# NVIDIA-Genomics-Research/GenomeWorks

Measured on AMD Instinct MI355X. Metric: cudapoa consensus GCUPS, 1024-window short-read batch (static band 256, 32 reads <= 1024 bp), higher is better.
Workload: dtype int16; 1 GPU; BASELINE configs[2]: cudapoa single-batch consensus, 1024 windows x 32 reads, backbone 960 bp, <=48 sub/24 ins/24 del, BatchConfig(1024,32,256,static_band), scores 8/-6/-8; windows_per_gpu=1024, cells_per_gpu=10990578176, parallelism=index-split x1

## Files before the change

genomeworks_amd/csrc/gwhip_poa.hip:

```cpp
#include <hip/hip_runtime.h>

#include <cstdio>
#include <cstdlib>
#include <cstring>
#include <string>

#include "poa_device.h"
#include "poa_full_device.h"
#include "poa_graph_device.h"
#include "poa_tb_device.h"

namespace gwhip
{

#ifndef GWHIP_POA_PART
thread_local std::string g_last_error;

static int fail(hipError_t e, const char* what)
{
    g_last_error = std::string(what) + ": " + hipGetErrorString(e);
    return (int)e;
}
static int fail_msg(int code, const std::string& msg)
{
// ... 177 lines not shown
        }
    }
    if (lane == 0) consensus[0] = 0;
    uint64_t cells = 0;
    int32_t node_count = len0;
    uint64_t phase_acc[kPhCount] = {0, 0, 0, 0, 0, 0};
    PhaseClock pc{(DBG && a.phase_cycles) ? phase_acc : nullptr, 0};
    wave_sync();
    pc.start();

    for (int32_t s = 1; s < (int32_t)wd.num_seqs; s++)
    {
        const int32_t seq_len = seq_lens[s];
        const int32_t adv     = ((s == 1 ? len0 : seq_lens[s - 1]) + 3) & ~3;
        sequence += adv;
        base_weights += adv;

        if (node_count >= c.max_nodes_per_graph)
        {
            if (lane == 0) { consensus[0] = kKernelError; consensus[1] = kNodeCountExceeded; }
            break;
        }
        pc.tick(kPhOther);
        build_rowinfo<IdT, RowT>(g, node_count, rowinfo, lane, LDS_TABLES ? reinterpret_cast<uint64_t*>(lds_code_tile) : nullptr);
        constexpr bool LDS_READ = LDS_TABLES && BM != GWHIP_FULL_BAND;
        const uint8_t* lds_read = lds_read_buf;
        if constexpr (LDS_READ)
        {
            typedef uint32_t StageVec __attribute__((ext_vector_type(4)));
            typedef StageVec StageVecA4 __attribute__((aligned(4)));
            static_assert(kReadLds % 16 == 0 && (kRingBytes + kRowInfoBytes) % 16 == 0, "16-byte fetches fill the LDS copy of the read");
            const int32_t stage_bytes = min(kReadLds, ((max(seq_len, kMaxAdaptiveBand) + 8) + 3) & ~3);
            for (int32_t i = lane * 16; i < stage_bytes; i += kWave * 16)
                *reinterpret_cast<StageVec*>(lds_read_buf + i) = *reinterpret_cast<const StageVecA4*>(sequence + i);
        }
        wave_sync();
        pc.tick(kPhRowInfo);
        const uint8_t* banded_read = LDS_READ ? lds_read : sequence;

        int32_t alen = 0;
        constexpr bool kTbPacked = TB && LDS_TABLES && std::is_same<ScoreT, int16_t>::value && std::is_same<TraceT, int16_t>::value;
        bool tb_handled = false;
        if constexpr (kTbPacked)
        {
            constexpr bool kAd = BM == GWHIP_ADAPTIVE_BAND_TRACEBACK;
            const bool adaptive_now = kAd && c.alignment_band_width < kMaxAdaptiveBand;
            auto packed = [&](auto ad_tag, int32_t rerun) -> int32_t {
// ... 20 lines not shown
            else
            alen = nw_banded_tb<ScoreT, IdT, RowT, TraceT, true>(g, rowinfo, node_count, sequence, seq_len, scores, a.L.scores_elems,
                                                           traceback, a.L.trace_elems, banded_buffer_size, alignment_graph,
                                                           alignment_read, c.alignment_band_width, c.max_banded_pred_distance,
                                                           c.gap_score, c.mismatch_score, c.match_score, 0, cells);
            if (alen == kShiftLeft || alen == kShiftRight)
                alen = nw_banded_tb<ScoreT, IdT, RowT, TraceT, true>(g, rowinfo, node_count, sequence, seq_len, scores, a.L.scores_elems,
                                                               traceback, a.L.trace_elems, banded_buffer_size, alignment_graph,
                                                               alignment_read, c.alignment_band_width, c.max_banded_pred_distance,
                                                               c.gap_score, c.mismatch_score, c.match_score, alen, cells);
        }
        else if (TB)
        {
            alen = nw_banded_tb<ScoreT, IdT, RowT, TraceT, false>(g, rowinfo, node_count, sequence, seq_len, scores, a.L.scores_elems,
                                                            traceback, a.L.trace_elems, banded_buffer_size, alignment_graph,
                                                            alignment_read, c.alignment_band_width, c.max_banded_pred_distance,
                                                            c.gap_score, c.mismatch_score, c.match_score, 0, cells);
        }
        else if (BM == GWHIP_ADAPTIVE_BAND && c.alignment_band_width < kMaxAdaptiveBand)
        {
            alen = nw_banded<ScoreT, IdT, RowT, true, LDS_READ, PV>(g, rowinfo, node_count, banded_read, lds_read, seq_len, scores, ring, ring_bytes,
                                                banded_buffer_size, alignment_graph, alignment_read, c.alignment_band_width,
                                                c.gap_score, c.mismatch_score, c.match_score, 0, cells, pc, debug_flags, codes, lds_code_tile, lds_read_window, lds_bs_ring,
                                                mw_args, mw_shared);
            if (alen == kShiftLeft || alen == kShiftRight)
                alen = nw_banded<ScoreT, IdT, RowT, true, LDS_READ, PV>(g, rowinfo, node_count, banded_read, lds_read, seq_len, scores, ring, ring_bytes,
                                                    banded_buffer_size, alignment_graph, alignment_read,
                                                    c.alignment_band_width, c.gap_score, c.mismatch_score, c.match_score,
                                                    alen, cells, pc, debug_flags, codes, lds_code_tile, lds_read_window, lds_bs_ring,
                                                    mw_args, mw_shared);
        }
        else if (BM == GWHIP_STATIC_BAND || BM == GWHIP_ADAPTIVE_BAND)
        {
            alen = nw_banded<ScoreT, IdT, RowT, false, LDS_READ, PV>(g, rowinfo, node_count, banded_read, lds_read, seq_len, scores, ring, ring_bytes,
                                                 banded_buffer_size, alignment_graph, alignment_read, c.alignment_band_width,
                                                 c.gap_score, c.mismatch_score, c.match_score, 0, cells, pc, debug_flags, codes, lds_code_tile, lds_read_window, lds_bs_ring);
        }
        else
        {
            bool full_handled = false;
            if constexpr (kFullPacked)
                alen = nw_full_packed<IdT>(g, rowinfo, node_count, sequence, seq_len, reinterpret_cast<int16_t*>(scores), wd.scores_width, full_moves,
                                           smem, kRingBytes, reinterpret_cast<const uint64_t*>(lds_code_tile), alignment_graph, alignment_read,
                                           c.gap_score, c.mismatch_score, c.match_score, cells, debug_flags, full_handled, pc);
            if (!full_handled)
                alen = nw_full<ScoreT, IdT, RowT>(g, rowinfo, node_count, sequence, seq_len, scores, wd.scores_width, ring, kRingBytes,
                                            alignment_graph, alignment_read, c.gap_score, c.mismatch_score, c.match_score, cells);
        }
        alen = (int32_t)(IdT)alen;

        uint8_t err = 0;
        if (alen == kNwLoopFailed) err = kLoopCountExceeded;
        else if (alen == kNwAdaptiveStorageFailed) err = kExceededAdaptiveBandedMatrixSize;
        else if (TB && alen == kNwTracebackBufferFailed) err = kExceededMaximumPredecessorDistance;
        else if (alen == kNwPipelineFailed || alen == kNwScoreWrapped) err = kGenericError;
        if (err)
        {
            if (lane == 0) { consensus[0] = kKernelError; consensus[1] = err; }
            break;
// ... 640 lines not shown
```

genomeworks_amd/csrc/poa_device.h:

```cpp
#pragma once
#include <hip/hip_runtime.h>
#include <stdint.h>

#include <type_traits>

#include "poa_layout.h"
#include "poa_pred_rows.h"

namespace gwhip
{

constexpr int kWave = 64;

template <typename T> struct Limits;
template <> struct Limits<int16_t> { static constexpr int32_t min = -32768; };
template <> struct Limits<int32_t> { static constexpr int32_t min = INT32_MIN; };

template <typename ScoreT> struct alignas(sizeof(ScoreT) * 4) Quad { ScoreT v[4]; };

template <typename ScoreT> __device__ __forceinline__ int32_t narrow_chk(int32_t v, bool& wrapped)
{
    const int32_t n = (int32_t)(ScoreT)v;
    if constexpr (sizeof(ScoreT) == 2) wrapped |= n != v;
    return n;
}

template <bool PACKED> struct RowInfo;
template <> struct alignas(8) RowInfo<true>
{
    uint64_t w;
// ... 689 lines not shown
    const uint64_t t_pp = psel == 6 ? clock64() : 0;
    if (aligned_nodes > 0 && (aligned_nodes & (kStage - 1)) != 0)
        flush_stage(aligned_nodes & ~(kStage - 1), aligned_nodes & (kStage - 1));
    if ((dbg & 2) && prof_acc && lane == 0) *prof_acc += (uint64_t)max(aligned_nodes, 0);
    if (aligned_nodes >= bound) aligned_nodes = kNwLoopFailed;
    wave_sync();
    for (int32_t k0 = lane; k0 < aligned_nodes; k0 += 4 * kWave)
    {
        int32_t pos[4], node[4];
#pragma unroll
        for (int u = 0; u < 4; u++) pos[u] = (k0 + u * kWave < aligned_nodes) ? alignment_graph[k0 + u * kWave] : -1;
#pragma unroll
        for (int u = 0; u < 4; u++) node[u] = (int32_t)g.sorted_poa[max(pos[u], 0)];
#pragma unroll
        for (int u = 0; u < 4; u++)
            if (pos[u] >= 0) alignment_graph[k0 + u * kWave] = node[u];
    }
    wave_sync();
    if (psel == 6) pacc += clock64() - t_pp;
    if (psel && lane == 0) *prof_acc += pacc;
    return aligned_nodes;
}

template <typename IdT, typename RowT>
__device__ __forceinline__ void build_rowinfo(const GraphView<IdT>& g, int32_t graph_count, RowT* rowinfo, int lane,
                                              uint64_t* xpred = nullptr)
{
    if (xpred != nullptr)
    {
#pragma unroll
        for (int q = 0; q < 4; q++) xpred[q * kWave + lane] = 0;
        wave_sync();
    }
    if (lane == 0) rowinfo[0].set(0, 0, false, 0, 0, 0);
    constexpr int kU = 4;
    for (int32_t r0 = 1 + lane; r0 <= graph_count; r0 += kU * kWave)
    {
        int32_t node[kU], cnt[kU], oc[kU], bas[kU], e0[kU], e1[kU], e2[kU], q0[kU], q1[kU], q2[kU];
        int32_t e3[kU], e4[kU], e5[kU], q3[kU] = {}, q4[kU] = {}, q5[kU] = {};
#pragma unroll
        for (int u = 0; u < kU; u++) node[u] = g.sorted_poa[min(r0 + u * kWave, graph_count) - 1];
#pragma unroll
        for (int u = 0; u < kU; u++)
        {
            cnt[u] = g.incoming_edge_count[node[u]];
            oc[u]  = g.outgoing_edge_count[node[u]];
            bas[u] = g.nodes[node[u]];
            e0[u]  = g.incoming_edges[(int64_t)node[u] * kEdges + 0];
            e1[u]  = g.incoming_edges[(int64_t)node[u] * kEdges + 1];
            e2[u]  = g.incoming_edges[(int64_t)node[u] * kEdges + 2];
        }
#pragma unroll
        for (int u = 0; u < kU; u++)
        {
            q0[u] = g.node_id_to_pos[(uint32_t)e0[u] < (uint32_t)graph_count ? e0[u] : 0];
            q1[u] = g.node_id_to_pos[(uint32_t)e1[u] < (uint32_t)graph_count ? e1[u] : 0];
            q2[u] = g.node_id_to_pos[(uint32_t)e2[u] < (uint32_t)graph_count ? e2[u] : 0];
            e3[u] = e4[u] = e5[u] = 0;
            if (xpred != nullptr && cnt[u] > 3)
            {
                e3[u] = g.incoming_edges[(int64_t)node[u] * kEdges + 3];
                e4[u] = g.incoming_edges[(int64_t)node[u] * kEdges + 4];
                e5[u] = g.incoming_edges[(int64_t)node[u] * kEdges + 5];
            }
        }
        if (xpred != nullptr)
        {
            bool any = false;
#pragma unroll
            for (int u = 0; u < kU; u++) any |= cnt[u] > 3;
            if (__ballot(any) != 0)
            {
#pragma unroll
                for (int u = 0; u < kU; u++)
                {
                    q3[u] = q4[u] = q5[u] = 0;
                    if (cnt[u] > 3)
                    {
                        q3[u] = g.node_id_to_pos[(uint32_t)e3[u] < (uint32_t)graph_count ? e3[u] : 0];
                        q4[u] = g.node_id_to_pos[(uint32_t)e4[u] < (uint32_t)graph_count ? e4[u] : 0];
                        q5[u] = g.node_id_to_pos[(uint32_t)e5[u] < (uint32_t)graph_count ? e5[u] : 0];
                    }
                }
            }
        }
#pragma unroll
        for (int u = 0; u < kU; u++)
        {
            const int32_t r = r0 + u * kWave;
            if (r <= graph_count)
            {
                RowT ri{};
                ri.set(bas[u], cnt[u], oc[u] == 0, cnt[u] > 0 ? q0[u] + 1 : 0, cnt[u] > 1 ? q1[u] + 1 : 0, cnt[u] > 2 ? q2[u] + 1 : 0);
                rowinfo[r] = ri;
                if (xpred != nullptr && cnt[u] > 3)
                    xpred[r & (kSideTableSlots - 1)] = xpred_entry(r, cnt[u], q3[u] + 1, q4[u] + 1, q5[u] + 1);
            }
        }
    }
}

template <typename ScoreT, typename IdT>
__device__ __forceinline__ void banded_forward_1pass(const GraphView<IdT>& g, const RowInfo<true>* rowinfo,
                                                     int32_t graph_count, const uint8_t* lds_read, ScoreT* scores,
                                                     ScoreT* ring, int32_t ring_rows, int32_t band_width,
                                                     int32_t max_column, int32_t gap_score, int32_t mismatch_score,
                                                     int32_t match_score, int32_t dbg, uint64_t* general_row_acc, bool& wrapped)
{
    const int lane          = threadIdx.x & (kWave - 1);
    const int32_t min_score = Limits<ScoreT>::min / 2;
    const int32_t stride    = band_width + kRightPad;
    const int32_t lane4     = lane * 4;
    uint64_t general_acc    = 0;
    const bool full_wave    = band_width == 256;
    const bool active       = lane4 < band_width;
    const int32_t K0 = (lane4 + 0) * gap_score, K1 = (lane4 + 1) * gap_score, K2 = (lane4 + 2) * gap_score,
                  K3 = (lane4 + 3) * gap_score;
    int32_t P0 = K0 + gap_score, P1 = K1 + gap_score, P2 = K2 + gap_score, P3 = K3 + gap_score;
    int32_t prev_bs = 0, prev_rel0 = 0;
    int32_t ring_slot = 0;
    bool hbm_dirty    = false;
    ScoreT* row_out   = scores;
// ... 814 lines not shown
        if ((uint32_t)tg < (uint32_t)band_width)
        {
            const int32_t rel = tg + 1;
            const int32_t slot_r = slot_now();
            lds_st_quad<ScoreT>(ring + slot_r * stride + rel + kRelShift, (ScoreT)H0, (ScoreT)H1, (ScoreT)H2, (ScoreT)H3);
            global_st_quad<ScoreT>(scores + (int64_t)r * stride + rel + kRelShift, (ScoreT)H0, (ScoreT)H1, (ScoreT)H2, (ScoreT)H3);
            if (codes) *reinterpret_cast<__attribute__((address_space(1))) uint32_t*>(codes + (int64_t)r * stride + rel + kRelShift) = code4;
        }
        if (first_block && lane == 0)
        {
            *(__attribute__((address_space(3))) ScoreT*)(ring + slot_now() * stride + kRelShift) = (ScoreT)rel0_val;
            scores[(int64_t)r * stride + kRelShift]                                          = (ScoreT)rel0_val;
        }
        publish(r, __builtin_amdgcn_readlane(H3, kWave - 1));
        if (sksel == 8 || (sksel == 11 && first_block)) skacc += clock64() - t_rb;
    }
    }
    if (sksel == 4) skacc += clock64() - t_pass;
    if (sksel && lane == 0) __hip_atomic_fetch_add(&shared->prof, (unsigned long long)skacc, __ATOMIC_RELAXED, __HIP_MEMORY_SCOPE_WORKGROUP);
    block_barrier();
    if (sksel && prof_out && lane == 0) *prof_out += shared->prof;
}

template <typename ScoreT, typename IdT, typename RowT, bool ADAPTIVE, bool LDS_READ, int PV = 0>
__device__ __forceinline__ int32_t nw_banded(const GraphView<IdT>& g, RowT* rowinfo, int32_t graph_count, const uint8_t* read,
                             const uint8_t* lds_read, int32_t read_length, ScoreT* scores, ScoreT* ring_base, int32_t ring_bytes,
                             float max_buffer_size, int32_t* alignment_graph, int32_t* alignment_read,
                             int32_t band_width, int32_t gap_score, int32_t mismatch_score, int32_t match_score,
                             int32_t rerun, uint64_t& cells, PhaseClock& pc, int32_t dbg = 0, uint8_t* codes = nullptr,
                             uint8_t* code_tile = nullptr, uint8_t* read_window = nullptr, int32_t* bs_ring = nullptr,
                             MwArgs<ScoreT>* mw_args = nullptr, MwShared* mw_shared = nullptr)
{
    const int lane              = threadIdx.x & (kWave - 1);
    const int32_t min_score     = Limits<ScoreT>::min / 2;
    const float gradient        = __fdiv_rn((float)(read_length + 1), (float)(graph_count + 1));
    const int32_t max_column    = read_length + 1;

    if (ADAPTIVE)
    {
        if ((double)gradient > 1.1)
            band_width = max(band_width, ((int32_t)((double)max_column * 0.08 * (double)gradient) + 127) & ~127);
        if ((double)gradient < 0.8)
            band_width = max(band_width, ((int32_t)((double)max_column * 0.1 / (double)gradient) + 127) & ~127);
        band_width = min(band_width, kMaxAdaptiveBand);
        if (band_width == kMaxAdaptiveBand && rerun != 0) return rerun;
    }
    int32_t band_shift = band_width / 2;
    if (ADAPTIVE)
    {
        if (rerun == kShiftLeft && band_width <= kMaxAdaptiveBand / 2)
        {
            band_width *= 2;
            band_shift = (int32_t)((double)band_shift * 2.5);
        }
        if (rerun == kShiftRight && band_width <= kMaxAdaptiveBand / 2)
        {
            band_width *= 2;
            band_shift = (int32_t)((double)band_shift * 1.5);
        }
        float required = __fmul_rn((float)graph_count, (float)(band_width + kRightPad));
        if (required > max_buffer_size) return kNwAdaptiveStorageFailed;
    }
    cells += (uint64_t)graph_count * (uint64_t)band_width;

    BandedCtx<ScoreT> b;
    b.scores     = scores;
    b.stride     = band_width + kRightPad;
    b.band_width = band_width;
    b.band_shift = band_shift;
    b.max_column = max_column;
    b.gradient   = gradient;
    b.min_score  = min_score;
    b.ring       = ring_base;
    b.ring_rows  = ring_bytes / (int32_t)(b.stride * sizeof(ScoreT));
    if (b.ring_rows < 2) b.ring_rows = 0;
    if (bs_ring != nullptr) b.ring_rows = min(b.ring_rows, 64);
    const int32_t stride = b.stride;
    const int32_t npass  = (band_width + 255) / 256;
    const bool reg_path  = (npass == 1);

    for (int32_t rel = lane; rel <= band_width; rel += kWave)
    {
        ScoreT v = (ScoreT)(rel * gap_score);
        scores[rel + kRelShift] = v;
        if (b.ring_rows) b.ring[rel + kRelShift] = v;
    }
    int32_t P0 = 0, P1 = 0, P2 = 0, P3 = 0;
    int32_t prev_bs   = 0;
    int32_t prev_rel0 = 0;
    if (reg_path)
    {
        int32_t c = 4 * lane;
        P0 = (ScoreT)((c + 1) * gap_score);
        P1 = (ScoreT)((c + 2) * gap_score);
        P2 = (ScoreT)((c + 3) * gap_score);
        P3 = (ScoreT)((c + 4) * gap_score);
        prev_rel0 = 0;
    }
    for (int32_t r = 1 + lane; r <= graph_count; r += kWave)
        rowinfo[r].set_bs(band_start_for_row(r, gradient, band_width, band_shift, max_column));
    bool hbm_dirty = true;
    wave_sync();
    hbm_dirty = false;
    auto bs_of = [&](int32_t row, int32_t r) -> int32_t {
        if (row == 0) return 0;
        if (bs_ring && b.ring_rows && r - row < b.ring_rows) return bs_ring[row % b.ring_rows];
        return uniform_row(rowinfo[row]).bs();
    };
    constexpr int32_t kWin = 4096, kWinStep = 1024;
    int32_t staged_end = 0;
    auto stage_read = [&](int32_t need_end) {
        while (staged_end < need_end)
        {
            for (int32_t i = lane * 4; i < kWinStep; i += kWave * 4)
            {
                const int32_t col = staged_end + i;
                const uint32_t v = col < read_length + 8 ? *reinterpret_cast<const uint32_t*>(read + col) : 0u;
                *reinterpret_cast<uint32_t*>(read_window + (col & (kWin - 1))) = v;
            }
            staged_end += kWinStep;
        }
        wave_sync();
    };

    constexpr bool kFastOk = std::is_same<RowT, RowInfo<true>>::value && LDS_READ;
    bool fast_done = false, codes_valid = false, moves_valid = false;
    bool packed_selective = false;
    bool wrapped = false;
    if constexpr (kFastOk && std::is_same<ScoreT, int16_t>::value)
    {
        const bool width_ok  = PV == 2 ? (band_width == 384 || band_width == 512) : (band_width == 256 || (PV == 1 && band_width == 128));
        const int32_t u_span = max(band_width, 256) * abs(gap_score);
        const bool packed_ok = width_ok && max_column >= band_width && ring_bytes >= kPkSlots * kPkSlotBytes &&
                               abs(gap_score) <= 30 && abs(match_score) <= 100 && abs(mismatch_score) <= 100 &&
                               codes != nullptr && !(dbg & 256) && ring_bytes >= kMtBytes &&
                               max(match_score, 0) * min(read_length, graph_count) + u_span + abs(match_score) <= 32767 &&
                               (graph_count + read_length) * min(min(gap_score, mismatch_score), 0) >= -32768 + 256 &&
                               min_score + 4 * min(min(gap_score, mismatch_score), 0) - u_span >= -32768;
        static_assert(kWdSlots * kWdSlotBytes <= kPkSlots * kPkSlotBytes, "the two-pass ring lives in the 256-column pass's ring region");
        if (packed_ok)
        {
            if constexpr (PV == 2)
            {
                if (band_width == 384)
                    banded_forward_moves_wide<IdT, 384>(g, rowinfo, graph_count, lds_read, scores, codes, reinterpret_cast<uint8_t*>(ring_base),
                                                        reinterpret_cast<const uint64_t*>(code_tile), max_column, gap_score, mismatch_score, match_score, dbg);
                else
                    banded_forward_moves_wide<IdT, 512>(g, rowinfo, graph_count, lds_read, scores, codes, reinterpret_cast<uint8_t*>(ring_base),
                                                        reinterpret_cast<const uint64_t*>(code_tile), max_column, gap_score, mismatch_score, match_score, dbg);
            }
            else if (band_width == 256)
            {
                banded_forward_moves<IdT, 256>(g, rowinfo, graph_count, lds_read, scores, codes, reinterpret_cast<uint8_t*>(ring_base),
                                               reinterpret_cast<const uint64_t*>(code_tile), max_column, gap_score, mismatch_score, match_score,
                                               dbg, pc.acc ? &pc.acc[kPhOther] : nullptr, (dbg & (1 << 25)) != 0);
                packed_selective = !(dbg & (1 << 25));
            }
            else if constexpr (PV == 1)
            {
                banded_forward_moves<IdT, 128>(g, rowinfo, graph_count, lds_read, scores, codes, reinterpret_cast<uint8_t*>(ring_base),
                                               reinterpret_cast<const uint64_t*>(code_tile), max_column, gap_score, mismatch_score, match_score,
                                               dbg, pc.acc ? &pc.acc[kPhOther] : nullptr, (dbg & (1 << 25)) != 0);
                packed_selective = !(dbg & (1 << 25));
            }
            fast_done   = true;
            moves_valid = true;
        }
    }
    if constexpr (kFastOk)
    {
        if (!fast_done && npass == 1 && b.ring_rows >= 2)
        {
            banded_forward_1pass<ScoreT, IdT>(g, rowinfo, graph_count, lds_read, scores, b.ring, b.ring_rows, band_width,
                                              max_column, gap_score, mismatch_score, match_score, dbg,
                                              pc.acc ? &pc.acc[kPhOther] : nullptr, wrapped);
            fast_done = true;
        }
    }
    if constexpr (!std::is_same<RowT, RowInfo<true>>::value)
    {
        const int32_t sk_rows = min(b.ring_rows, (int32_t)(200.0f / (gradient + 1.0f)));
        if (!fast_done && mw_args != nullptr && npass >= 2 && sk_rows >= kSkLead + 3 && !(dbg & (1 << 18)))
        {
            MwArgs<ScoreT> A;
            A.op = 1;
// ... 331 lines not shown
```

genomeworks_amd/csrc/poa_forward_moves.h:

```cpp
#pragma once

#include "poa_forward_row_operands.h"

namespace gwhip
{

constexpr int kKindShift = 60;
constexpr uint32_t kMoveHoriz = 1;

__device__ __forceinline__ uint32_t pk_mad_u16_vsv(uint32_t a, uint32_t s, uint32_t c)
{
    uint32_t d;
    asm("v_pk_mad_u16 %0, %1, %2, %3" : "=v"(d) : "v"(a), "s"(s), "v"(c));
    return d;
}
__device__ __forceinline__ uint32_t pk_mad_u16_vvs(uint32_t a, uint32_t b, uint32_t s)
{
    uint32_t d;
    asm("v_pk_mad_u16 %0, %1, %2, %3" : "=v"(d) : "v"(a), "v"(b), "s"(s));
    return d;
}
__device__ __forceinline__ void gstore_nt_u64(void* p, uint32_t lo, uint32_t hi)
{
    u32x2 v;
// ... 93 lines not shown
            {
                int32_t e[kB], q[kB];
#pragma unroll
                for (int u = 0; u < kB; u++) e[u] = (int32_t)g.incoming_edges[edges + min(k0 + u, cnt - 1)];
#pragma unroll
                for (int u = 0; u < kB; u++) q[u] = (int32_t)g.node_id_to_pos[e[u]];
#pragma unroll
                for (int u = 0; u < kB; u++) mark(q[u] + 1);
            }
        }
    }
    wave_sync();
}
__device__ __forceinline__ bool row_recompute_safe(uint64_t w)
{
    return ((uint32_t)(w >> kKindShift) & 7u) >= 4u || ((w >> 8) & 0x3fu) > 3u || ((w >> 15) & 0x1ffu) == 0u;
}

template <typename IdT, int BW>
__device__ __forceinline__ void banded_forward_moves(const GraphView<IdT>& g, RowInfo<true>* rowinfo, int32_t graph_count,
                                                     const uint8_t* lds_read, int16_t* scores, uint8_t* moves, uint8_t* ring,
                                                     const uint64_t* xpred, int32_t max_column, int32_t gap_score,
                                                     int32_t mismatch_score, int32_t match_score, int32_t dbg,
                                                     uint64_t* prof_acc, bool store_all = true)
{
    const bool abl       = (dbg & (1 << 14)) != 0;
    const bool st_scores = !(abl && (dbg & (1 << 26))), st_moves = !(abl && (dbg & (1 << 27)));
    const bool ab_ring = !(abl && (dbg & (1 << 20))), ab_guard = !(abl && (dbg & (1 << 19))), ab_scan = !(abl && (dbg & (1 << 18))),
               ab_moves = !(abl && (dbg & (1 << 17))), ab_rows = !(abl && (dbg & (1 << 16)));
    const int32_t ksel = prof_acc ? ((dbg >> 28) & 7) - 1 : -1;
    const bool kfine   = (dbg & (1 << 13)) != 0;
    const bool kcount  = (dbg & (1 << 12)) != 0;
    uint64_t kacc      = 0;
    auto kselected = [&](uint32_t dk) -> bool { return ksel == (int32_t)((kfine || dk < kDkRingThree) ? dk : (uint32_t)kDkRingTwo); };
    const bool ksel_prev = kselected(kDkPrev), ksel_moved = kselected(kDkPrevMoved), ksel_one = kselected(kDkRingOne),
               ksel_two = kselected(kDkRingTwo), ksel_three = kselected(kDkRingThree), ksel_many = kselected(kDkRingMany),
               ksel_general = kselected(kDkGeneral);
    static_assert(kRowOpSlots == kPkSlots && kRowOpSlotBytes == kPkSlotBytes, "the row operands fold the ring's geometry in");
    static_assert(BW == 128 || BW == 256, "band widths of the packed pass");
    constexpr int32_t band_width = BW;
    constexpr int32_t stride     = band_width + kRightPad;
    constexpr int kBandLanes     = BW / kCellsPerLane;
    const int lane               = threadIdx.x & (kWave - 1);
    const bool band_lane         = lane < kBandLanes;
    const int32_t lane4 = lane * 4, lane8 = lane * 8;
    const int32_t min_score = Limits<int16_t>::min / 2;

    const bool time_prologue  = prof_acc != nullptr && ksel < 0 && kcount;
    const uint64_t t_prologue = time_prologue ? clock64() : 0;
    const int32_t first_moved = classify_kinds(rowinfo, graph_count, lane, xpred, dbg);
    wave_sync();
    static_assert(kPkSlots * kPkSlotBytes >= 4096 * (int)sizeof(uint16_t), "the ring region holds the list of left-over rows (rows <= 4095)");
    mark_score_rows<IdT>(g, rowinfo, graph_count, lane, store_all, reinterpret_cast<uint16_t*>(ring), xpred);
    if (time_prologue && lane == 0) *prof_acc += clock64() - t_prologue;

    const uint32_t MIN2   = pin_vgpr(pk_dup(min_score));
    const uint32_t SENT2  = pin_vgpr(pk_dup(kPkSentinel));
    const uint32_t GAP2   = pin_vgpr(pk_dup(gap_score));
    const uint32_t MAT2   = pin_vgpr(pk_dup(match_score));
    const uint32_t DIF2   = pin_vgpr(pk_dup(mismatch_score - match_score));
    const uint32_t ONE2   = pin_vgpr(0x00010001u);
    const uint32_t THREE2 = pin_vgpr(0x00030003u);
    const uint32_t NEG1   = pin_vgpr(0xffffffffu);
    const uint32_t K01 = pk_make((lane4 + 0) * gap_score, (lane4 + 1) * gap_score);
    const uint32_t K23 = pk_make((lane4 + 2) * gap_score, (lane4 + 3) * gap_score);
    const uint32_t ring_base = lds_addr(ring);
    const uint32_t read_base = lds_addr(lds_read);
    const uint32_t guard_off  = lane < 16 ? (uint32_t)(2 * BW) : (lane == 16 ? (uint32_t)-136 : (uint32_t)(120 - 16 * lane));
    const bool is_lane16      = lane == 16;
    const bool is_lane63      = lane == kBandLanes - 1;
    const uint32_t move_keep  = lane == 0 ? 0xffffff00u : 0xffffffffu;
    const uint32_t GUARD_HI_MIN = pin_vgpr(is_lane16 ? (((uint32_t)kPkSentinel & 0xffffu) | ((uint32_t)min_score << 16)) : pk_dup(kPkSentinel));
    const uint32_t S0X_MIN      = (uint32_t)min_score << 16;

    uint32_t P01 = pk_make((lane4 + 1) * gap_score, (lane4 + 2) * gap_score);
    uint32_t P23 = pk_make((lane4 + 3) * gap_score, (lane4 + 4) * gap_score);
// ... 434 lines not shown
```

Measured before the change: 451.1 GCUPS.

## Fold row classification and score-row marking into the row-table build

When the static or adaptive banded int16 packed pass will run, the row table is built in a new pass that also computes each row's band start, its kind and its mark bit, and collects a list of rows whose predecessors need marking. The forward-moves kernel then skips its separate classify_kinds and mark_score_rows prologue passes. This saves two extra sweeps over the row table plus their wave syncs for each read. In exchange it duplicates the classification rules in a new header, which must stay in step with the original, and it adds atomic ORs into the LDS row words.

```diff
diff --git a/genomeworks_amd/csrc/gwhip_poa.hip b/genomeworks_amd/csrc/gwhip_poa.hip
--- a/genomeworks_amd/csrc/gwhip_poa.hip
+++ b/genomeworks_amd/csrc/gwhip_poa.hip
@@ -223,7 +223,26 @@
             break;
         }
         pc.tick(kPhOther);
-        build_rowinfo<IdT, RowT>(g, node_count, rowinfo, lane, LDS_TABLES ? reinterpret_cast<uint64_t*>(lds_code_tile) : nullptr);
+        constexpr bool kFinishTable = LDS_TABLES && std::is_same<ScoreT, int16_t>::value && PV <= 1 &&
+                                      (BM == GWHIP_STATIC_BAND || BM == GWHIP_ADAPTIVE_BAND);
+        RowTableFinish fin{};
+        if constexpr (kFinishTable)
+        {
+            const bool adaptive_now = BM == GWHIP_ADAPTIVE_BAND && c.alignment_band_width < kMaxAdaptiveBand;
+            fin.plan = adaptive_now ? band_plan<true>(node_count, seq_len, c.alignment_band_width, 0, banded_buffer_size)
+                                    : band_plan<false>(node_count, seq_len, c.alignment_band_width, 0, banded_buffer_size);
+            const bool finish = fin.plan.early == 0 && !row_table_old_passes(debug_flags) && fin.plan.max_column <= kFinishMaxColumn &&
+                                packed_pass_ok<PV>(fin.plan.band_width, fin.plan.max_column, seq_len, node_count, ring_bytes, c.gap_score,
+                                                   c.mismatch_score, c.match_score, codes != nullptr, debug_flags);
+            const bool time_stores = pc.acc != nullptr && (debug_flags & (7 << 28)) == 0 && (debug_flags & (3 << 12)) == (3 << 12);
+            if (__builtin_amdgcn_readfirstlane((int32_t)finish) != 0)
+                build_rowinfo_finished<IdT>(g, node_count, rowinfo, lane, reinterpret_cast<uint64_t*>(lds_code_tile), reinterpret_cast<uint64_t*>(smem),
+                                            fin, time_stores ? &pc.acc[kPhOther] : nullptr);
+            else
+                build_rowinfo<IdT, RowT>(g, node_count, rowinfo, lane, reinterpret_cast<uint64_t*>(lds_code_tile));
+        }
+        else
+            build_rowinfo<IdT, RowT>(g, node_count, rowinfo, lane, LDS_TABLES ? reinterpret_cast<uint64_t*>(lds_code_tile) : nullptr);
         constexpr bool LDS_READ = LDS_TABLES && BM != GWHIP_FULL_BAND;
         const uint8_t* lds_read = lds_read_buf;
         if constexpr (LDS_READ)
@@ -290,7 +309,7 @@
             alen = nw_banded<ScoreT, IdT, RowT, true, LDS_READ, PV>(g, rowinfo, node_count, banded_read, lds_read, seq_len, scores, ring, ring_bytes,
                                                 banded_buffer_size, alignment_graph, alignment_read, c.alignment_band_width,
                                                 c.gap_score, c.mismatch_score, c.match_score, 0, cells, pc, debug_flags, codes, lds_code_tile, lds_read_window, lds_bs_ring,
-                                                mw_args, mw_shared);
+                                                mw_args, mw_shared, kFinishTable ? &fin : nullptr);
             if (alen == kShiftLeft || alen == kShiftRight)
                 alen = nw_banded<ScoreT, IdT, RowT, true, LDS_READ, PV>(g, rowinfo, node_count, banded_read, lds_read, seq_len, scores, ring, ring_bytes,
                                                     banded_buffer_size, alignment_graph, alignment_read,
@@ -302,7 +321,8 @@
         {
             alen = nw_banded<ScoreT, IdT, RowT, false, LDS_READ, PV>(g, rowinfo, node_count, banded_read, lds_read, seq_len, scores, ring, ring_bytes,
                                                  banded_buffer_size, alignment_graph, alignment_read, c.alignment_band_width,
-                                                 c.gap_score, c.mismatch_score, c.match_score, 0, cells, pc, debug_flags, codes, lds_code_tile, lds_read_window, lds_bs_ring);
+                                                 c.gap_score, c.mismatch_score, c.match_score, 0, cells, pc, debug_flags, codes, lds_code_tile, lds_read_window, lds_bs_ring,
+                                                 nullptr, nullptr, kFinishTable ? &fin : nullptr);
         }
         else
         {
diff --git a/genomeworks_amd/csrc/poa_device.h b/genomeworks_amd/csrc/poa_device.h
--- a/genomeworks_amd/csrc/poa_device.h
+++ b/genomeworks_amd/csrc/poa_device.h
@@ -6,6 +6,7 @@
 
 #include "poa_layout.h"
 #include "poa_pred_rows.h"
+#include "poa_row_finish.h"
 
 namespace gwhip
 {
@@ -741,6 +742,63 @@
     return aligned_nodes;
 }
 
+constexpr int kRowChunks = 4;
+struct RowChunkLoads
+{
+    int32_t cnt[kRowChunks], oc[kRowChunks], bas[kRowChunks];
+    int32_t q0[kRowChunks], q1[kRowChunks], q2[kRowChunks], q3[kRowChunks], q4[kRowChunks], q5[kRowChunks];
+};
+template <typename IdT>
+__device__ __forceinline__ void load_row_chunks(const GraphView<IdT>& g, int32_t graph_count, int32_t r0, bool side, RowChunkLoads& L)
+{
+    constexpr int kU = kRowChunks;
+    int32_t node[kU], e0[kU], e1[kU], e2[kU], e3[kU], e4[kU], e5[kU];
+#pragma unroll
+    for (int u = 0; u < kU; u++) node[u] = g.sorted_poa[min(r0 + u * kWave, graph_count) - 1];
+#pragma unroll
+    for (int u = 0; u < kU; u++)
+    {
+        L.cnt[u] = g.incoming_edge_count[node[u]];
+        L.oc[u]  = g.outgoing_edge_count[node[u]];
+        L.bas[u] = g.nodes[node[u]];
+        e0[u]    = g.incoming_edges[(int64_t)node[u] * kEdges + 0];
+        e1[u]    = g.incoming_edges[(int64_t)node[u] * kEdges + 1];
+        e2[u]    = g.incoming_edges[(int64_t)node[u] * kEdges + 2];
+    }
+#pragma unroll
+    for (int u = 0; u < kU; u++)
+    {
+        L.q0[u] = g.node_id_to_pos[(uint32_t)e0[u] < (uint32_t)graph_count ? e0[u] : 0];
+        L.q1[u] = g.node_id_to_pos[(uint32_t)e1[u] < (uint32_t)graph_count ? e1[u] : 0];
+        L.q2[u] = g.node_id_to_pos[(uint32_t)e2[u] < (uint32_t)graph_count ? e2[u] : 0];
+        e3[u] = e4[u] = e5[u] = 0;
+        L.q3[u] = L.q4[u] = L.q5[u] = 0;
+        if (side && L.cnt[u] > 3)
+        {
+            e3[u] = g.incoming_edges[(int64_t)node[u] * kEdges + 3];
+            e4[u] = g.incoming_edges[(int64_t)node[u] * kEdges + 4];
+            e5[u] = g.incoming_edges[(int64_t)node[u] * kEdges + 5];
+        }
+    }
+    if (side)
+    {
+        bool any = false;
+#pragma unroll
+        for (int u = 0; u < kU; u++) any |= L.cnt[u] > 3;
+        if (__ballot(any) != 0)
+        {
+#pragma unroll
+            for (int u = 0; u < kU; u++)
+                if (L.cnt[u] > 3)
+                {
+                    L.q3[u] = g.node_id_to_pos[(uint32_t)e3[u] < (uint32_t)graph_count ? e3[u] : 0];
+                    L.q4[u] = g.node_id_to_pos[(uint32_t)e4[u] < (uint32_t)graph_count ? e4[u] : 0];
+                    L.q5[u] = g.node_id_to_pos[(uint32_t)e5[u] < (uint32_t)graph_count ? e5[u] : 0];
+                }
+        }
+    }
+}
+
 template <typename IdT, typename RowT>
 __device__ __forceinline__ void build_rowinfo(const GraphView<IdT>& g, int32_t graph_count, RowT* rowinfo, int lane,
                                               uint64_t* xpred = nullptr)
@@ -752,57 +810,11 @@
         wave_sync();
     }
     if (lane == 0) rowinfo[0].set(0, 0, false, 0, 0, 0);
-    constexpr int kU = 4;
+    constexpr int kU = kRowChunks;
     for (int32_t r0 = 1 + lane; r0 <= graph_count; r0 += kU * kWave)
     {
-        int32_t node[kU], cnt[kU], oc[kU], bas[kU], e0[kU], e1[kU], e2[kU], q0[kU], q1[kU], q2[kU];
-        int32_t e3[kU], e4[kU], e5[kU], q3[kU] = {}, q4[kU] = {}, q5[kU] = {};
-#pragma unroll
-        for (int u = 0; u < kU; u++) node[u] = g.sorted_poa[min(r0 + u * kWave, graph_count) - 1];
-#pragma unroll
-        for (int u = 0; u < kU; u++)
-        {
-            cnt[u] = g.incoming_edge_count[node[u]];
-            oc[u]  = g.outgoing_edge_count[node[u]];
-            bas[u] = g.nodes[node[u]];
-            e0[u]  = g.incoming_edges[(int64_t)node[u] * kEdges + 0];
-            e1[u]  = g.incoming_edges[(int64_t)node[u] * kEdges + 1];
-            e2[u]  = g.incoming_edges[(int64_t)node[u] * kEdges + 2];
-        }
-#pragma unroll
-        for (int u = 0; u < kU; u++)
-        {
-            q0[u] = g.node_id_to_pos[(uint32_t)e0[u] < (uint32_t)graph_count ? e0[u] : 0];
-            q1[u] = g.node_id_to_pos[(uint32_t)e1[u] < (uint32_t)graph_count ? e1[u] : 0];
-            q2[u] = g.node_id_to_pos[(uint32_t)e2[u] < (uint32_t)graph_count ? e2[u] : 0];
-            e3[u] = e4[u] = e5[u] = 0;
-            if (xpred != nullptr && cnt[u] > 3)
-            {
-                e3[u] = g.incoming_edges[(int64_t)node[u] * kEdges + 3];
-                e4[u] = g.incoming_edges[(int64_t)node[u] * kEdges + 4];
-                e5[u] = g.incoming_edges[(int64_t)node[u] * kEdges + 5];
-            }
-        }
-        if (xpred != nullptr)
-        {
-            bool any = false;
-#pragma unroll
-            for (int u = 0; u < kU; u++) any |= cnt[u] > 3;
-            if (__ballot(any) != 0)
-            {
-#pragma unroll
-                for (int u = 0; u < kU; u++)
-                {
-                    q3[u] = q4[u] = q5[u] = 0;
-                    if (cnt[u] > 3)
-                    {
-                        q3[u] = g.node_id_to_pos[(uint32_t)e3[u] < (uint32_t)graph_count ? e3[u] : 0];
-                        q4[u] = g.node_id_to_pos[(uint32_t)e4[u] < (uint32_t)graph_count ? e4[u] : 0];
-                        q5[u] = g.node_id_to_pos[(uint32_t)e5[u] < (uint32_t)graph_count ? e5[u] : 0];
-                    }
-                }
-            }
-        }
+        RowChunkLoads L;
+        load_row_chunks<IdT>(g, graph_count, r0, xpred != nullptr, L);
 #pragma unroll
         for (int u = 0; u < kU; u++)
         {
@@ -810,13 +822,166 @@
             if (r <= graph_count)
             {
                 RowT ri{};
-                ri.set(bas[u], cnt[u], oc[u] == 0, cnt[u] > 0 ? q0[u] + 1 : 0, cnt[u] > 1 ? q1[u] + 1 : 0, cnt[u] > 2 ? q2[u] + 1 : 0);
+                ri.set(L.bas[u], L.cnt[u], L.oc[u] == 0, L.cnt[u] > 0 ? L.q0[u] + 1 : 0, L.cnt[u] > 1 ? L.q1[u] + 1 : 0, L.cnt[u] > 2 ? L.q2[u] + 1 : 0);
                 rowinfo[r] = ri;
-                if (xpred != nullptr && cnt[u] > 3)
-                    xpred[r & (kSideTableSlots - 1)] = xpred_entry(r, cnt[u], q3[u] + 1, q4[u] + 1, q5[u] + 1);
-            }
-        }
-    }
+                if (xpred != nullptr && L.cnt[u] > 3)
+                    xpred[r & (kSideTableSlots - 1)] = xpred_entry(r, L.cnt[u], L.q3[u] + 1, L.q4[u] + 1, L.q5[u] + 1);
+            }
+        }
+    }
+}
+
+struct BandPlan
+{
+    float gradient;
+    int32_t max_column, band_width, band_shift;
+    int32_t early;
+};
+template <bool ADAPTIVE>
+__device__ __forceinline__ BandPlan band_plan(int32_t graph_count, int32_t read_length, int32_t band_width, int32_t rerun, float max_buffer_size)
+{
+    BandPlan p;
+    p.gradient   = __fdiv_rn((float)(read_length + 1), (float)(graph_count + 1));
+    p.max_column = read_length + 1;
+    p.early      = 0;
+    if (ADAPTIVE)
+    {
+        if ((double)p.gradient > 1.1)
+            band_width = max(band_width, ((int32_t)((double)p.max_column * 0.08 * (double)p.gradient) + 127) & ~127);
+        if ((double)p.gradient < 0.8)
+            band_width = max(band_width, ((int32_t)((double)p.max_column * 0.1 / (double)p.gradient) + 127) & ~127);
+        band_width = min(band_width, kMaxAdaptiveBand);
+        if (band_width == kMaxAdaptiveBand && rerun != 0) p.early = rerun;
+    }
+    int32_t band_shift = band_width / 2;
+    if (ADAPTIVE && p.early == 0)
+    {
+        if (rerun == kShiftLeft && band_width <= kMaxAdaptiveBand / 2)
+        {
+            band_width *= 2;
+            band_shift = (int32_t)((double)band_shift * 2.5);
+        }
+        if (rerun == kShiftRight && band_width <= kMaxAdaptiveBand / 2)
+        {
+            band_width *= 2;
+            band_shift = (int32_t)((double)band_shift * 1.5);
+        }
+        float required = __fmul_rn((float)graph_count, (float)(band_width + kRightPad));
+        if (required > max_buffer_size) p.early = kNwAdaptiveStorageFailed;
+    }
+    p.band_width = band_width;
+    p.band_shift = band_shift;
+    return p;
+}
+
+struct RowTableFinish
+{
+    BandPlan plan;
+    bool finished;
+    bool marks_done;
+    int32_t first_moved;
+};
+constexpr int kFinishMarkerSlots = 1024;
+template <typename IdT>
+__device__ __forceinline__ void build_rowinfo_finished(const GraphView<IdT>& g, int32_t graph_count, RowInfo<true>* rowinfo, int lane,
+                                                       uint64_t* xpred, uint64_t* markers, RowTableFinish& fin, uint64_t* timer = nullptr)
+{
+    static_assert(kRowChunks * kWave == kSideTableSlots, "the rows of one side-table slot belong to one lane and one chunk");
+    static_assert(kFinishCellsPerLane == kCellsPerLane, "poa_row_finish.h restates the band rounding");
+    const BandParams bp{fin.plan.gradient, fin.plan.band_width, fin.plan.band_shift, fin.plan.max_column};
+#pragma unroll
+    for (int q = 0; q < 4; q++) xpred[q * kWave + lane] = 0;
+    wave_sync();
+    if (lane == 0) rowinfo[0].set(0, 0, false, 0, 0, 0);
+    constexpr int kU    = kRowChunks;
+    uint32_t slot_taken = 0;
+    int32_t first_moved = graph_count + 1;
+    int32_t n_mark      = 0;
+    uint64_t ticks      = 0;
+    const uint64_t lanes_below = (1ull << lane) - 1ull;
+    for (int32_t it = (graph_count + kU * kWave - 1) / (kU * kWave) - 1; it >= 0; it--)
+    {
+        const int32_t r0 = 1 + lane + it * kU * kWave;
+        RowChunkLoads L;
+        load_row_chunks<IdT>(g, graph_count, r0, true, L);
+        uint64_t t0 = 0;
+        if (timer)
+        {
+            __builtin_amdgcn_s_waitcnt(0);
+            t0 = clock64();
+        }
+#pragma unroll
+        for (int u = 0; u < kU; u++)
+        {
+            const int32_t r = r0 + u * kWave;
+            bool marker     = false;
+            uint64_t entry  = 0;
+            if (r <= graph_count)
+            {
+                const int32_t cnt = L.cnt[u];
+                const bool sink   = L.oc[u] == 0;
+                const bool many   = cnt > kTablePreds;
+                const bool kept   = many && ((slot_taken >> u) & 1u) == 0;
+                const int32_t p0 = L.q0[u] + 1, p1 = L.q1[u] + 1, p2 = L.q2[u] + 1, p3 = L.q3[u] + 1, p4 = L.q4[u] + 1, p5 = L.q5[u] + 1;
+                const int32_t bs    = finish_row_bs(r, bp);
+                const uint32_t kind = finish_row_kind(r, cnt, bs, p0, p1, p2, p3, p4, p5, kept, bp);
+                rowinfo[r].w        = finish_table_word(L.bas[u], cnt, sink, bs, p0, p1, p2, kind);
+                if (kept) xpred[r & (kSideTableSlots - 1)] = xpred_entry(r, cnt, p3, p4, p5);
+                if (many) slot_taken |= 1u << u;
+                if (bs > 0) first_moved = min(first_moved, r);
+                marker = finish_row_marks_others(kind, cnt);
+                entry  = finish_marker_entry(r, p3, p4, p5);
+            }
+            const uint64_t m = __ballot(marker);
+            if (m != 0)
+            {
+                const int32_t at = n_mark + __popcll(m & lanes_below);
+                if (marker && at < kFinishMarkerSlots) markers[at] = entry;
+                n_mark += __popcll(m);
+            }
+        }
+        if (timer) ticks += clock64() - t0;
+    }
+    uint64_t t1 = 0;
+    if (timer) t1 = clock64();
+    for (int off = 32; off > 0; off >>= 1) first_moved = min(first_moved, __shfl_xor(first_moved, off));
+    wave_sync();
+    const bool fits = n_mark <= kFinishMarkerSlots;
+    if (fits)
+    {
+        auto mark = [&](int32_t row) {
+            __hip_atomic_fetch_or(reinterpret_cast<uint32_t*>(&rowinfo[row].w) + 1, 0x80000000u, __ATOMIC_RELAXED, __HIP_MEMORY_SCOPE_WORKGROUP);
+        };
+        for (int32_t i = lane; i < n_mark; i += kWave)
+        {
+            const uint64_t e  = markers[i];
+            const int32_t r   = finish_marker_row(e);
+            const uint64_t w  = rowinfo[r].w;
+            const int32_t cnt = table_pred_count(w);
+            const int32_t n   = min(cnt, kSideTablePreds);
+            for (int32_t k = 0; k < n; k++) mark(finish_marker_pred(w, e, k));
+            if (cnt > kSideTablePreds)
+            {
+                constexpr int kB    = 6;
+                const int64_t edges = (int64_t)g.sorted_poa[r - 1] * kEdges;
+                for (int32_t k0 = kSideTablePreds; k0 < cnt; k0 += kB)
+                {
+                    int32_t ee[kB], qq[kB];
+#pragma unroll
+                    for (int u = 0; u < kB; u++) ee[u] = (int32_t)g.incoming_edges[edges + min(k0 + u, cnt - 1)];
+#pragma unroll
+                    for (int u = 0; u < kB; u++) qq[u] = (int32_t)g.node_id_to_pos[ee[u]];
+#pragma unroll
+                    for (int u = 0; u < kB; u++) mark(qq[u] + 1);
+                }
+            }
+        }
+        wave_sync();
+    }
+    fin.finished    = true;
+    fin.marks_done  = fits;
+    fin.first_moved = __builtin_amdgcn_readfirstlane(first_moved);
+    if (timer && lane == 0) *timer += ticks + (clock64() - t1);
 }
 
 template <typename ScoreT, typename IdT>
@@ -1677,6 +1842,26 @@
     if (sksel && prof_out && lane == 0) *prof_out += shared->prof;
 }
 
+template <int PV>
+__device__ __forceinline__ bool packed_pass_ok(int32_t band_width, int32_t max_column, int32_t read_length, int32_t graph_count, int32_t ring_bytes,
+                                               int32_t gap_score, int32_t mismatch_score, int32_t match_score, bool have_moves, int32_t dbg)
+{
+    const int32_t min_score = Limits<int16_t>::min / 2;
+    const bool width_ok  = PV == 2 ? (band_width == 384 || band_width == 512) : (band_width == 256 || (PV == 1 && band_width == 128));
+    const int32_t u_span = max(band_width, 256) * abs(gap_score);
+    return width_ok && max_column >= band_width && ring_bytes >= kPkSlots * kPkSlotBytes &&
+           abs(gap_score) <= 30 && abs(match_score) <= 100 && abs(mismatch_score) <= 100 &&
+           have_moves && !(dbg & 256) && ring_bytes >= kMtBytes &&
+           max(match_score, 0) * min(read_length, graph_count) + u_span + abs(match_score) <= 32767 &&
+           (graph_count + read_length) * min(min(gap_score, mismatch_score), 0) >= -32768 + 256 &&
+           min_score + 4 * min(min(gap_score, mismatch_score), 0) - u_span >= -32768;
+}
+
+__device__ __forceinline__ bool row_table_old_passes(int32_t dbg)
+{
+    return dbg < 0 || (dbg & ((1 << 9) | (1 << 10) | (1 << 11) | (1 << 15) | (1 << 25))) != 0 || ((dbg & (1 << 30)) != 0 && (dbg & (1 << 13)) == 0);
+}
+
 template <typename ScoreT, typename IdT, typename RowT, bool ADAPTIVE, bool LDS_READ, int PV = 0>
 __device__ __forceinline__ int32_t nw_banded(const GraphView<IdT>& g, RowT* rowinfo, int32_t graph_count, const uint8_t* read,
                              const uint8_t* lds_read, int32_t read_length, ScoreT* scores, ScoreT* ring_base, int32_t ring_bytes,
@@ -1684,38 +1869,17 @@
                              int32_t band_width, int32_t gap_score, int32_t mismatch_score, int32_t match_score,
                              int32_t rerun, uint64_t& cells, PhaseClock& pc, int32_t dbg = 0, uint8_t* codes = nullptr,
                              uint8_t* code_tile = nullptr, uint8_t* read_window = nullptr, int32_t* bs_ring = nullptr,
-                             MwArgs<ScoreT>* mw_args = nullptr, MwShared* mw_shared = nullptr)
+                             MwArgs<ScoreT>* mw_args = nullptr, MwShared* mw_shared = nullptr, const RowTableFinish* fin = nullptr)
 {
     const int lane              = threadIdx.x & (kWave - 1);
     const int32_t min_score     = Limits<ScoreT>::min / 2;
-    const float gradient        = __fdiv_rn((float)(read_length + 1), (float)(graph_count + 1));
-    const int32_t max_column    = read_length + 1;
-
-    if (ADAPTIVE)
-    {
-        if ((double)gradient > 1.1)
-            band_width = max(band_width, ((int32_t)((double)max_column * 0.08 * (double)gradient) + 127) & ~127);
-        if ((double)gradient < 0.8)
-            band_width = max(band_width, ((int32_t)((double)max_column * 0.1 / (double)gradient) + 127) & ~127);
-        band_width = min(band_width, kMaxAdaptiveBand);
-        if (band_width == kMaxAdaptiveBand && rerun != 0) return rerun;
-    }
-    int32_t band_shift = band_width / 2;
-    if (ADAPTIVE)
-    {
-        if (rerun == kShiftLeft && band_width <= kMaxAdaptiveBand / 2)
-        {
-            band_width *= 2;
-            band_shift = (int32_t)((double)band_shift * 2.5);
-        }
-        if (rerun == kShiftRight && band_width <= kMaxAdaptiveBand / 2)
-        {
-            band_width *= 2;
-            band_shift = (int32_t)((double)band_shift * 1.5);
-        }
-        float required = __fmul_rn((float)graph_count, (float)(band_width + kRightPad));
-        if (required > max_buffer_size) return kNwAdaptiveStorageFailed;
-    }
+    const BandPlan plan         = (fin != nullptr && rerun == 0) ? fin->plan : band_plan<ADAPTIVE>(graph_count, read_length, band_width, rerun, max_buffer_size);
+    if (plan.early != 0) return plan.early;
+    const float gradient        = plan.gradient;
+    const int32_t max_column    = plan.max_column;
+    band_width                  = plan.band_width;
+    const int32_t band_shift    = plan.band_shift;
+    const bool table_finished   = fin != nullptr && rerun == 0 && fin->finished;
     cells += (uint64_t)graph_count * (uint64_t)band_width;
 
     BandedCtx<ScoreT> b;
@@ -1752,8 +1916,9 @@
         P3 = (ScoreT)((c + 4) * gap_score);
         prev_rel0 = 0;
     }
-    for (int32_t r = 1 + lane; r <= graph_count; r += kWave)
-        rowinfo[r].set_bs(band_start_for_row(r, gradient, band_width, band_shift, max_column));
+    if (!table_finished)
+        for (int32_t r = 1 + lane; r <= graph_count; r += kWave)
+            rowinfo[r].set_bs(band_start_for_row(r, gradient, band_width, band_shift, max_column));
     bool hbm_dirty = true;
     wave_sync();
     hbm_dirty = false;
@@ -1784,14 +1949,8 @@
     bool wrapped = false;
     if constexpr (kFastOk && std::is_same<ScoreT, int16_t>::value)
     {
-        const bool width_ok  = PV == 2 ? (band_width == 384 || band_width == 512) : (band_width == 256 || (PV == 1 && band_width == 128));
-        const int32_t u_span = max(band_width, 256) * abs(gap_score);
-        const bool packed_ok = width_ok && max_column >= band_width && ring_bytes >= kPkSlots * kPkSlotBytes &&
-                               abs(gap_score) <= 30 && abs(match_score) <= 100 && abs(mismatch_score) <= 100 &&
-                               codes != nullptr && !(dbg & 256) && ring_bytes >= kMtBytes &&
-                               max(match_score, 0) * min(read_length, graph_count) + u_span + abs(match_score) <= 32767 &&
-                               (graph_count + read_length) * min(min(gap_score, mismatch_score), 0) >= -32768 + 256 &&
-                               min_score + 4 * min(min(gap_score, mismatch_score), 0) - u_span >= -32768;
+        const bool packed_ok = packed_pass_ok<PV>(band_width, max_column, read_length, graph_count, ring_bytes, gap_score, mismatch_score,
+                                                  match_score, codes != nullptr, dbg);
         static_assert(kWdSlots * kWdSlotBytes <= kPkSlots * kPkSlotBytes, "the two-pass ring lives in the 256-column pass's ring region");
         if (packed_ok)
         {
@@ -1808,14 +1967,16 @@
             {
                 banded_forward_moves<IdT, 256>(g, rowinfo, graph_count, lds_read, scores, codes, reinterpret_cast<uint8_t*>(ring_base),
                                                reinterpret_cast<const uint64_t*>(code_tile), max_column, gap_score, mismatch_score, match_score,
-                                               dbg, pc.acc ? &pc.acc[kPhOther] : nullptr, (dbg & (1 << 25)) != 0);
+                                               dbg, pc.acc ? &pc.acc[kPhOther] : nullptr, (dbg & (1 << 25)) != 0,
+                                               table_finished ? fin->first_moved : -1, table_finished && fin->marks_done);
                 packed_selective = !(dbg & (1 << 25));
             }
             else if constexpr (PV == 1)
             {
                 banded_forward_moves<IdT, 128>(g, rowinfo, graph_count, lds_read, scores, codes, reinterpret_cast<uint8_t*>(ring_base),
                                                reinterpret_cast<const uint64_t*>(code_tile), max_column, gap_score, mismatch_score, match_score,
-                                               dbg, pc.acc ? &pc.acc[kPhOther] : nullptr, (dbg & (1 << 25)) != 0);
+                                               dbg, pc.acc ? &pc.acc[kPhOther] : nullptr, (dbg & (1 << 25)) != 0,
+                                               table_finished ? fin->first_moved : -1, table_finished && fin->marks_done);
                 packed_selective = !(dbg & (1 << 25));
             }
             fast_done   = true;
diff --git a/genomeworks_amd/csrc/poa_forward_moves.h b/genomeworks_amd/csrc/poa_forward_moves.h
--- a/genomeworks_amd/csrc/poa_forward_moves.h
+++ b/genomeworks_amd/csrc/poa_forward_moves.h
@@ -139,8 +139,12 @@
                                                      const uint8_t* lds_read, int16_t* scores, uint8_t* moves, uint8_t* ring,
                                                      const uint64_t* xpred, int32_t max_column, int32_t gap_score,
                                                      int32_t mismatch_score, int32_t match_score, int32_t dbg,
-                                                     uint64_t* prof_acc, bool store_all = true)
-{
+                                                     uint64_t* prof_acc, bool store_all = true, int32_t finished_first_moved = -1,
+                                                     bool marks_done = false)
+{
+    static_assert(kFinishMaxDist == kPkMaxDist && kFinishGuardCols == kPkGuardCols && kFinishKindGeneral == 4,
+                  "poa_row_finish.h restates classify_kinds' rule");
+    static_assert(kFinishMarkerSlots * (int)sizeof(uint64_t) <= kPkSlots * kPkSlotBytes, "the ring region holds the marker list");
     const bool abl       = (dbg & (1 << 14)) != 0;
     const bool st_scores = !(abl && (dbg & (1 << 26))), st_moves = !(abl && (dbg & (1 << 27)));
     const bool ab_ring = !(abl && (dbg & (1 << 20))), ab_guard = !(abl && (dbg & (1 << 19))), ab_scan = !(abl && (dbg & (1 << 18))),
@@ -163,12 +167,13 @@
     const int32_t lane4 = lane * 4, lane8 = lane * 8;
     const int32_t min_score = Limits<int16_t>::min / 2;
 
-    const bool time_prologue  = prof_acc != nullptr && ksel < 0 && kcount;
+    const bool time_prologue  = prof_acc != nullptr && ksel < 0 && kcount && !kfine;
     const uint64_t t_prologue = time_prologue ? clock64() : 0;
-    const int32_t first_moved = classify_kinds(rowinfo, graph_count, lane, xpred, dbg);
-    wave_sync();
+    const bool table_finished = finished_first_moved >= 0;
+    const int32_t first_moved = table_finished ? finished_first_moved : classify_kinds(rowinfo, graph_count, lane, xpred, dbg);
+    if (!table_finished) wave_sync();
     static_assert(kPkSlots * kPkSlotBytes >= 4096 * (int)sizeof(uint16_t), "the ring region holds the list of left-over rows (rows <= 4095)");
-    mark_score_rows<IdT>(g, rowinfo, graph_count, lane, store_all, reinterpret_cast<uint16_t*>(ring), xpred);
+    if (!(table_finished && marks_done)) mark_score_rows<IdT>(g, rowinfo, graph_count, lane, store_all, reinterpret_cast<uint16_t*>(ring), xpred);
     if (time_prologue && lane == 0) *prof_acc += clock64() - t_prologue;
 
     const uint32_t MIN2   = pin_vgpr(pk_dup(min_score));
diff --git a/genomeworks_amd/csrc/poa_row_finish.h b/genomeworks_amd/csrc/poa_row_finish.h
--- /dev/null
+++ b/genomeworks_amd/csrc/poa_row_finish.h
@@ -0,0 +1,86 @@
+#pragma once
+
+#include <cstdint>
+
+#include "poa_pred_rows.h"
+
+#if defined(__HIPCC__)
+#define GWHIP_ROW_FINISH_FN __host__ __device__ inline
+#else
+#define GWHIP_ROW_FINISH_FN inline
+#endif
+
+namespace gwhip
+{
+
+constexpr int kFinishCellsPerLane = 4;
+constexpr int kFinishGuardCols    = 60;
+constexpr int kFinishMaxDist      = 7;
+constexpr uint32_t kFinishKindGeneral = 4;
+
+struct BandParams
+{
+    float gradient;
+    int32_t band_width, band_shift, max_column;
+};
+
+GWHIP_ROW_FINISH_FN int32_t finish_band_start(int32_t row, const BandParams& b)
+{
+#if defined(__HIP_DEVICE_COMPILE__)
+    const int32_t diagonal_index = (int32_t)__fmul_rn((float)row, b.gradient);
+#else
+    const float product          = (float)row * b.gradient;
+    const int32_t diagonal_index = (int32_t)product;
+#endif
+    int32_t start_pos = diagonal_index - b.band_shift > 0 ? diagonal_index - b.band_shift : 0;
+    if (b.max_column - b.band_width < start_pos)
+        start_pos = b.max_column - b.band_width + kFinishCellsPerLane > 0 ? b.max_column - b.band_width + kFinishCellsPerLane : 0;
+    return start_pos & ~(kFinishCellsPerLane - 1);
+}
+GWHIP_ROW_FINISH_FN int32_t finish_table_bs(int32_t bs) { return (int32_t)(((uint32_t)bs >> 2) & 0x1ffu) << 2; }
+GWHIP_ROW_FINISH_FN int32_t finish_row_bs(int32_t row, const BandParams& b) { return row == 0 ? 0 : finish_table_bs(finish_band_start(row, b)); }
+
+constexpr int32_t kFinishMaxColumn = 2047;
+
+GWHIP_ROW_FINISH_FN uint32_t finish_row_kind(int32_t r, int32_t cnt, int32_t bs, int32_t p0, int32_t p1, int32_t p2, int32_t p3, int32_t p4,
+                                             int32_t p5, bool slot_kept, const BandParams& b, int32_t maxd = kFinishMaxDist)
+{
+    if (cnt < 1 || !(cnt <= kTablePreds || (cnt <= kSideTablePreds && slot_kept))) return kFinishKindGeneral;
+    const int32_t first = p0 & 0xfff;
+    int32_t nearest = first, farthest = first;
+    auto take = [&](int32_t p) { p &= 0xfff; nearest = p > nearest ? p : nearest; farthest = p < farthest ? p : farthest; };
+    if (cnt > 1) take(p1);
+    if (cnt > 2) take(p2);
+    if (cnt > 3)
+    {
+        take(p3);
+        if (cnt > 4) take(p4);
+        if (cnt > 5) take(p5);
+    }
+    const int32_t pbs = finish_row_bs(farthest, b);
+    const bool ok     = r - nearest >= 1 && r - farthest <= maxd && (bs - pbs) <= kFinishGuardCols && (bs == 0 || pbs > 0);
+    if (!ok) return kFinishKindGeneral;
+    if (cnt > 1) return 3u;
+    return (r - first == 1 && pbs == bs) ? 0u : ((r - first == 1 && bs - pbs == kFinishCellsPerLane) ? 1u : 2u);
+}
+
+GWHIP_ROW_FINISH_FN bool finish_row_marks_others(uint32_t kind, int32_t cnt) { return kind >= kFinishKindGeneral || cnt > kTablePreds; }
+GWHIP_ROW_FINISH_FN bool finish_row_own_mark(uint32_t kind, int32_t cnt, bool sink) { return finish_row_marks_others(kind, cnt) || sink; }
+
+GWHIP_ROW_FINISH_FN uint64_t finish_table_word(int32_t base, int32_t cnt, bool sink, int32_t bs, int32_t p0, int32_t p1, int32_t p2, uint32_t kind)
+{
+    return table_word(base, cnt, sink, cnt > 0 ? p0 : 0, cnt > 1 ? p1 : 0, cnt > 2 ? p2 : 0) | ((uint64_t)(((uint32_t)bs >> 2) & 0x1ffu) << 15) |
+           ((uint64_t)kind << 60) | ((uint64_t)(finish_row_own_mark(kind, cnt, sink) ? 1 : 0) << 63);
+}
+
+GWHIP_ROW_FINISH_FN uint64_t finish_marker_entry(int32_t row, int32_t p3, int32_t p4, int32_t p5)
+{
+    return (uint64_t)(row & 0xfff) | ((uint64_t)(p3 & 0xfff) << 12) | ((uint64_t)(p4 & 0xfff) << 24) | ((uint64_t)(p5 & 0xfff) << 36);
+}
+GWHIP_ROW_FINISH_FN int32_t finish_marker_row(uint64_t e) { return (int32_t)(e & 0xfffu); }
+GWHIP_ROW_FINISH_FN int32_t finish_marker_pred(uint64_t w, uint64_t e, int32_t k)
+{
+    return k < kTablePreds ? table_pred_row(w, k) : (int32_t)((e >> (12 * (k - 2))) & 0xfffu);
+}
+
+}
```

New measurement: 453.0 GCUPS (median of 6 runs). No clear change (+0.4%).
